# morrislab/rnascan

Hardware: AMD Instinct MI355X
Metric: scored windows/sec (seq+struct, w=12) (higher is better)
Workload: dtype f64

## Files before the change

### include/pfmscan.h

```cpp
#ifndef PFMSCAN_H
#define PFMSCAN_H

#include <stdint.h>

#ifdef __cplusplus
extern "C" {
#endif

#define PFMSCAN_ABI_VERSION 14
#define PFMSCAN_NCODE   8
#define PFMSCAN_SEP     7
#define PFMSCAN_NSTRUCT 7
#define PFMSCAN_MAX_M   64
#define PFMSCAN_MAX_WIDTH 4096

#define PFMSCAN_OK          0
#define PFMSCAN_E_BADARG   -1
#define PFMSCAN_E_BADSHAPE -2
#define PFMSCAN_E_OOM      -3
#define PFMSCAN_E_HIP      -4
#define PFMSCAN_E_CAPACITY -5

#define PFMSCAN_PROFILE_NONE 0
#define PFMSCAN_PROFILE_F32  1
#define PFMSCAN_PROFILE_F64  2

typedef struct pfmscan_ctx pfmscan_ctx;
typedef struct pfmscan_motif pfmscan_motif;

int pfmscan_abi_version(void);

int pfmscan_ctx_create(int device, pfmscan_ctx **out);
// ... 166 lines not shown
int pfmscan_library_sum_thresholds(const double *letter_tables, const double *struct_pssms,
                                   int n_motifs, int m, const double *thr_seq,
                                   const double *thr_sum, double row_sum_max, double *thr_eff_out);

int pfmscan_library_create_letters(pfmscan_ctx *ctx, const double *seq_tables,
                                   const double *struct_tables, int n_motifs, int m,
                                   pfmscan_library **out);
int pfmscan_library_hits_letters_dev(pfmscan_ctx *ctx, pfmscan_library *lib,
                                     const uint8_t *d_codes, const uint8_t *d_codes2, int64_t n_pos,
                                     const double *thr_seq, const double *thr_struct, int64_t capacity,
                                     int64_t *d_hit_pos, int32_t *d_hit_motif, float *d_hit_seq,
                                     double *d_hit_struct, uint64_t *d_hit_count, void *stream);
int pfmscan_library_hits_letters_host(pfmscan_ctx *ctx, pfmscan_library *lib,
                                      const uint8_t *codes, const uint8_t *codes2, int64_t n_pos,
                                      const double *thr_seq, const double *thr_struct, int64_t capacity,
                                      int64_t *hit_pos, int32_t *hit_motif, float *hit_seq,
                                      double *hit_struct, int64_t *n_hits);

int pfmscan_debug_credit_table(const double *letter_table, int m, double thr_seq, int bits,
                               uint16_t *credits, double *slack);

int pfmscan_debug_library8_credits(const double *letter_table, int m, double thr, uint16_t *credits, double *slack);

int pfmscan_debug_credit8_table(const double *letter_table, int m, double thr, uint16_t *credits, int *mode);

#define PFMSCAN_UPLOAD_RUNTIME 0
#define PFMSCAN_UPLOAD_STAGED  1
int pfmscan_set_upload_mode(pfmscan_ctx *ctx, int mode);
int pfmscan_upload_source_file(pfmscan_ctx *ctx, const void *base, size_t length, const char *path, int64_t file_offset);
int pfmscan_upload_source_file_checked(pfmscan_ctx *ctx, const void *base, size_t length, const char *path,
                                       int64_t file_offset, int64_t st_dev, int64_t st_ino, int64_t st_size);

int pfmscan_dotbracket_annotate_dev(pfmscan_ctx *ctx, const uint8_t *d_in, uint8_t *d_out, int64_t n_pos,
                                    const uint8_t *map, int64_t *d_counts, int64_t *first_bad, void *stream);
int pfmscan_dotbracket_stage(pfmscan_ctx *ctx, const uint8_t *codes, int64_t n_pos, int which, const uint8_t *map,
                             int64_t *counts, int64_t *first_bad);
int pfmscan_dotbracket_annotate_host(pfmscan_ctx *ctx, const uint8_t *in, uint8_t *out, int64_t n_pos,
                                     const uint8_t *map, int64_t *counts, int64_t *first_bad);

#define PFMSCAN_MAX_COVER 1024
#define PFMSCAN_AVG_OK         0
#define PFMSCAN_AVG_DOTBRACKET 1
#define PFMSCAN_AVG_UNCOVERED  2
#define PFMSCAN_AVG_COVER      3
#define PFMSCAN_AVG_BAD_TABLE  4
int pfmscan_average_dev(pfmscan_ctx *ctx, const uint8_t *d_letters, int64_t n_letters, const int64_t *d_frag_off,
// ... 84 lines not shown
```

### rnascan_amd/_lib.py

```python
import ctypes
import importlib.util
import os
import sys

import numpy as np

HERE = os.path.dirname(os.path.abspath(__file__))
LIB_PATH = os.environ.get("PFMSCAN_LIB") or os.path.join(HERE, "libpfmscan.so")

OK = 0
E_BADARG, E_BADSHAPE, E_OOM, E_HIP, E_CAPACITY = -1, -2, -3, -4, -5
PROFILE_NONE, PROFILE_F32, PROFILE_F64 = 0, 1, 2
SEP = 7
NCODE = 8
NSTRUCT = 7
MAX_M = 64
MAX_WIDTH = 4096
ABI_VERSION = 14

SYMBOLS = [
    "pfmscan_abi_version", "pfmscan_ctx_create", "pfmscan_ctx_destroy", "pfmscan_last_error",
    "pfmscan_device_info", "pfmscan_synchronize", "pfmscan_motif_create", "pfmscan_motif_destroy",
    "pfmscan_pwm_calculate", "pfmscan_scan_dev", "pfmscan_scan_letters_f64_dev", "pfmscan_hits_dev",
    "pfmscan_scan_host", "pfmscan_scan_letters_f64_host", "pfmscan_hits_host", "pfmscan_time_scan_dev",
    "pfmscan_stage", "pfmscan_scan_staged", "pfmscan_hits_staged", "pfmscan_hits_adaptive_dev",
    "pfmscan_library_create", "pfmscan_library_destroy", "pfmscan_library_info", "pfmscan_library_hits_dev",
    "pfmscan_library_hits_staged", "pfmscan_library_hits_host", "pfmscan_library_hits_pipeline_host", "pfmscan_debug_credit_table",
    "pfmscan_library_create_letters", "pfmscan_library_hits_letters_dev", "pfmscan_library_hits_letters_host", "pfmscan_debug_library8_credits",
    "pfmscan_debug_credit8_table",
    "pfmscan_hits_pipeline_host", "pfmscan_staged_positions",
    "pfmscan_hits_letters_f64_dev", "pfmscan_hits_letters_f64_staged", "pfmscan_hits_letters_f64_host",
    "pfmscan_hits_pair_dev", "pfmscan_stage_codes2", "pfmscan_hits_pair_staged", "pfmscan_hits_pair_host", "pfmscan_round_decimals",
    "pfmscan_set_upload_mode", "pfmscan_upload_source_file", "pfmscan_upload_source_file_checked", "pfmscan_fasta_lone_cr", "pfmscan_count_bytes", "pfmscan_fasta_index", "pfmscan_fasta_ids", "pfmscan_gather_spans", "pfmscan_fasta_encode", "pfmscan_tsv_format", "pfmscan_profile_parse", "pfmscan_tsv_number",
    "pfmscan_place_alloc", "pfmscan_place_free", "pfmscan_place_note", "pfmscan_place_trim",
    "pfmscan_dotbracket_annotate_dev", "pfmscan_dotbracket_stage", "pfmscan_dotbracket_annotate_host",
    "pfmscan_average_dev", "pfmscan_average_host", "pfmscan_average_stage", "pfmscan_fragment_ids",
    "pfmscan_profile_colsums_dev", "pfmscan_profile_colsums_host", "pfmscan_profile_colsums_staged",
    "pfmscan_hits_sum_dev", "pfmscan_hits_sum_staged", "pfmscan_hits_sum_host", "pfmscan_hits_sum_pipeline_host",
    "pfmscan_library_hits_sum_dev", "pfmscan_library_hits_sum_staged", "pfmscan_library_hits_sum_host",
    "pfmscan_profile_row_bound_dev", "pfmscan_profile_row_bound_staged", "pfmscan_library_sum_thresholds",
]
MAX_COVER = 1024
AVG_OK, AVG_DOTBRACKET, AVG_UNCOVERED, AVG_COVER, AVG_BAD_TABLE = range(5)
TSV_CONST, TSV_I64, TSV_F32, TSV_F64, TSV_INDEXED, TSV_FIXED, TSV_WINDOW, TSV_SPAN = range(8)


class TsvColumn(ctypes.Structure):
    _fields_ = [("kind", ctypes.c_int32), ("reserved", ctypes.c_int32), ("data", ctypes.c_void_p),
                ("aux", ctypes.c_void_p), ("blob", ctypes.c_void_p), ("width", ctypes.c_int64)]



# ... 1110 lines not shown
    tj = np.ascontiguousarray(np.broadcast_to(np.asarray(thr_sum, dtype=np.float64), (n,)))
    out = np.empty(n, dtype=np.float64)
    rc = L.pfmscan_library_sum_thresholds(_ptr(T), _ptr(P), n, m, _ptr(ts), _ptr(tj), float(row_sum_max), _ptr(out))
    if rc != OK:
        raise ValueError("pfmscan_library_sum_thresholds: bad argument")
    return out


def library8_credits(letter_table, thr):
    L = load()
    T = np.ascontiguousarray(letter_table, dtype=np.float64)
    if T.ndim != 2 or T.shape[1] != NCODE:
        raise ValueError("letter_table must be [m][8]")
    rows = (T.shape[0] + 3) // 4 * 4
    out = np.zeros((rows, 8), dtype=np.uint16)
    slack = ctypes.c_double(0.0)
    L.pfmscan_debug_library8_credits.argtypes = [ctypes.c_void_p, ctypes.c_int, ctypes.c_double, ctypes.c_void_p, ctypes.POINTER(ctypes.c_double)]
    rc = L.pfmscan_debug_library8_credits(_ptr(T), T.shape[0], float(thr), _ptr(out), ctypes.byref(slack))
    if rc != OK:
        raise ValueError("pfmscan_debug_library8_credits: bad argument")
    return out, slack.value


def credit8_table(letter_table, thr):
    L = load()
    T = np.ascontiguousarray(letter_table, dtype=np.float64)
    if T.ndim != 2 or T.shape[1] != NCODE:
        raise ValueError("letter_table must be [m][8]")
    out = np.zeros((T.shape[0], 8), dtype=np.uint16)
    mode = ctypes.c_int(0)
    rc = L.pfmscan_debug_credit8_table(_ptr(T), T.shape[0], float(thr), _ptr(out), ctypes.byref(mode))
    if rc != OK:
        raise ValueError("pfmscan_debug_credit8_table: bad argument")
    return out, mode.value


def _stream_args(motif, codes, profile):
    if motif.has_letters:
        if codes is None:
            raise ValueError("motif has a letter table: codes required")
        codes = np.ascontiguousarray(codes, dtype=np.uint8)
        n = codes.size
    dt = PROFILE_NONE
    if motif.has_struct:
        if profile is None:
            raise ValueError("motif has a structure PSSM: profile required")
# ... 16 lines not shown
```

### rnascan_amd/build.py

```python
import os
import re
import shutil
import subprocess
import sys
import tempfile
from concurrent.futures import ThreadPoolExecutor

HERE = os.path.dirname(os.path.abspath(__file__))
CSRC = os.path.join(HERE, "csrc")
OBJ = os.path.join(CSRC, "_obj")
LIB = os.path.join(HERE, "libpfmscan.so")
SOURCES = ["pfmscan_kernels.hip", "pfmscan_letters8.hip", "pfmscan_letters_fixed.hip", "pfmscan_api.hip", "pfmscan_hits.hip", "pfmscan_sort.hip", "pfmscan_library.hip", "pfmscan_library_api.hip", "pfmscan_proflib.hip", "pfmscan_profile_fixed.hip", "pfmscan_place.hip",
           "pfmscan_pipeline.hip", "pfmscan_ingest.hip", "pfmscan_upload.hip", "pfmscan_dotbracket.hip", "pfmscan_average.hip", "pfmscan_background.hip", "pfmscan_rowbound.hip"]
HEADERS = ["pfmscan_internal.hpp", "pfmscan_ctx.hpp", "pfmscan_hits.hpp", "pfmscan_hitqueue.hpp", "pfmscan_device.hpp", "pfmscan_profile.hpp", "pfmscan_exact.hpp", os.path.join("..", "..", "include", "pfmscan.h")]
DEPS = SOURCES + HEADERS
FLAGS = ["-O3", "--offload-arch=gfx950", "-std=c++17", "-fPIC", "-fno-fast-math", "-Wall"]


def hipcc_path():
    for cand in (os.environ.get("HIPCC"), shutil.which("hipcc"), "/opt/rocm/bin/hipcc"):
        if cand and os.path.exists(cand):
            return cand
    raise RuntimeError("hipcc not found (set HIPCC or install ROCm under /opt/rocm)")


def stale():
    if not os.path.exists(LIB):
        return True
    t = os.path.getmtime(LIB)
    return any(os.path.getmtime(os.path.join(CSRC, d)) > t for d in DEPS)


def _obj_stale(src, obj):
    if not os.path.exists(obj):
        return True
    t = os.path.getmtime(obj)
    return any(os.path.getmtime(os.path.join(CSRC, d)) > t for d in [src] + HEADERS)
# ... 70 lines not shown
```

### rnascan_amd/csrc/pfmscan_internal.hpp

```cpp
#pragma once
#include <hip/hip_runtime.h>
#include <stdint.h>
#include <atomic>
#include "../../include/pfmscan.h"

namespace pfmscan {

struct CredCache {
    double thr = __builtin_nan("");
    int mode = 0;
    uint16_t cr[16 * 16];
};

struct Cred8Cache {
    double thr = __builtin_nan("");
    int mode = 0;
    uint16_t cr[32 * 8];
};

struct ScanArgs {
    const uint8_t *codes;
    const void *profile;
    int profile_dtype;
    int64_t n_pos;
// ... 142 lines not shown
constexpr int PROFILE_LETTERS2 = 100;
__host__ __device__ constexpr int lib8_rows(int m) { return (m + 3) / 4 * 4; }
size_t lib8_group_bytes(int m);
size_t lib8_lds_bytes(int m, int ng);
int lib8_pick_ng(int want_groups, int max_groups);
hipError_t launch_library8(const LibArgs &a, int n_cu, hipStream_t stream);

struct ProfLibArgs {
    const void *profile;
    int profile_dtype;
    int64_t n_pos;
    const double *pssm;
    const double *thr;
    double struct_band;
    const int32_t *finite;
    int n_motifs, m, motif_base;
    int64_t pos_offset;
    int64_t capacity;
    int hit_shards;
    int64_t *hit_pos;
    int32_t *hit_motif;
    double *hit_struct;
    unsigned long long *hit_count;
};
hipError_t launch_profile_library(const ProfLibArgs &a, hipStream_t stream);
int64_t profile_library_tile();

hipError_t sort_temp_bytes(int64_t total, int key_bits, size_t *bytes);
hipError_t launch_gather_sorted(const GatherArgs &g, hipStream_t stream);

}
```

### rnascan_amd/csrc/pfmscan_library_api.hip

```cpp
#include <algorithm>
#include <cmath>
#include <cstdlib>
#include <cstring>
#include <new>
#include <string>
#include <vector>

#include "pfmscan_hits.hpp"

using namespace pfmscan;

namespace {

struct LibPass {
    int motif_base = 0, n_real = 0, nmp = 0, ng = 0;
    int ng_real = 0;
    size_t pairs_off = 0;
    size_t letters_off = 0;
    size_t pssm_off = 0;
    size_t thr_off = 0;
};

}

double pfmscan::build_credits(const double *pairsum, int npair, double thr, uint16_t *out, int bits, int nent)
{
    std::fill(out, out + (size_t)npair * nent, (uint16_t)0);
    if (thr == INFINITY) return 0.0;
    const int half = 1 << (bits - 1);
    const int V = std::min(half - 1, (half - 1) / std::max(npair - 1, 1));
    const int X = (npair - 1) * V + 1;
// ... 39 lines not shown
        }
    return q * npair;
}

void pfmscan::pair_sums(const double *T, int m, double *out)
{
    const int npair = (m + 1) / 2;
    for (int t = 0; t < npair; ++t)
        for (int c0 = 0; c0 < 4; ++c0)
            for (int c1 = 0; c1 < 4; ++c1)
                out[t * 16 + (c0 | c1 << 2)] = T[(2 * t) * 8 + c0] + (2 * t + 1 < m ? T[(2 * t + 1) * 8 + c1] : 0.0);
}

struct pfmscan_library {
    pfmscan_ctx *ctx = nullptr;
    int n = 0, m = 0, npair = 0, np_bucket = 8;
    bool has_struct = false;
    bool has_letters = true;
    bool pair = false;
    bool letters8 = false;
    std::vector<double> rows8;
    double *d_pssm_rows = nullptr;
    int32_t *d_finite = nullptr;
    bool all_finite = false;
    double struct_band = 0.0;
    std::vector<double> pairsum;
    std::vector<LibPass> passes;
    uint16_t *d_pairs = nullptr;
    double *d_letters = nullptr, *d_pssm = nullptr, *d_thr = nullptr;
    size_t pairs_elems = 0, thr_elems = 0;
    std::vector<uint16_t> h_pairs;
    std::vector<double> h_thr;
    std::vector<double> cur_seq, cur_struct, eps;
    std::vector<double> h_letters, h_pssm;
    std::vector<double> band;
    std::vector<double> cur_eff, cur_sum;
    bool thr_valid = false;
};

static int lib_fail(pfmscan_ctx *ctx, int code, const std::string &msg) { return fail(ctx, code, msg); }

extern "C" {

static int create_seq_library(pfmscan_ctx *ctx, const double *letter_tables, const double *struct_pssms, int ncol, int n_motifs, int m,
                              pfmscan_library **out);

// ... 7 lines not shown
        return lib_fail(ctx, PFMSCAN_E_BADSHAPE, "PFM width " + std::to_string(m) + " outside 1.." + std::to_string(PFMSCAN_MAX_M));
    if (!letter_tables) {
        HIP_TRY(ctx, hipSetDevice(ctx->device));
        pfmscan_library *lib = new (std::nothrow) pfmscan_library();
        if (!lib) return lib_fail(ctx, PFMSCAN_E_OOM, "out of host memory");
        lib->ctx = ctx;
        lib->n = n_motifs;
        lib->m = m;
        lib->has_struct = true;
        lib->has_letters = false;
        for (int k = 0; k < n_motifs; ++k) lib->struct_band = std::max(lib->struct_band, struct_band(struct_pssms + (size_t)k * m * 7, m));
        std::vector<int32_t> fin((size_t)n_motifs, 1);
        for (int k = 0; k < n_motifs; ++k)
            for (int i = 0; i < m * 7; ++i)
                if (!std::isfinite(struct_pssms[(size_t)k * m * 7 + i])) fin[(size_t)k] = 0;
        if (std::getenv("PFMSCAN_FORCE_GENERIC")) std::fill(fin.begin(), fin.end(), 0);
        const size_t cells = (size_t)n_motifs * m * 7;
        hipError_t e = hipMalloc((void **)&lib->d_pssm_rows, cells * 8);
        if (e == hipSuccess) e = hipMemcpy(lib->d_pssm_rows, struct_pssms, cells * 8, hipMemcpyHostToDevice);
        if (e == hipSuccess) e = hipMalloc((void **)&lib->d_finite, (size_t)n_motifs * 4);
        if (e == hipSuccess) e = hipMemcpy(lib->d_finite, fin.data(), (size_t)n_motifs * 4, hipMemcpyHostToDevice);
        if (e == hipSuccess) e = hipMalloc((void **)&lib->d_thr, (size_t)n_motifs * 8);
        lib->thr_elems = (size_t)n_motifs;
        if (e != hipSuccess) {
            pfmscan_library_destroy(lib);
            return fail_hip(ctx, e, "uploading the library tables");
        }
        *out = lib;
        return PFMSCAN_OK;
    }
    return create_seq_library(ctx, letter_tables, struct_pssms, 7, n_motifs, m, out);
}

}

static int create_seq_library(pfmscan_ctx *ctx, const double *letter_tables, const double *struct_pssms, int ncol, int n_motifs, int m,
                              pfmscan_library **out)
{
    for (int64_t i = 0; i < (int64_t)n_motifs * m; ++i)
        for (int c = 4; c < 8; ++c)
            if (!std::isnan(letter_tables[i * 8 + c]))
                return lib_fail(ctx, PFMSCAN_E_BADSHAPE, "library scans need a 4-letter alphabet: columns 4..7 of every letter table must be NaN");
    HIP_TRY(ctx, hipSetDevice(ctx->device));
    pfmscan_library *lib = new (std::nothrow) pfmscan_library();
    if (!lib) return lib_fail(ctx, PFMSCAN_E_OOM, "out of host memory");
    lib->ctx = ctx;
// ... 151 lines not shown
{
    if (!ctx || !out || !struct_tables) return lib_fail(ctx, PFMSCAN_E_BADARG, "pfmscan_library_create_letters: NULL argument");
    *out = nullptr;
    if (n_motifs < 1 || n_motifs > 65535) return lib_fail(ctx, PFMSCAN_E_BADSHAPE, "library size outside 1..65535");
    if (m < 1 || m > PFMSCAN_MAX_M)
        return lib_fail(ctx, PFMSCAN_E_BADSHAPE, "PFM width " + std::to_string(m) + " outside 1.." + std::to_string(PFMSCAN_MAX_M));
    for (int64_t i = 0; i < (int64_t)n_motifs * m; ++i)
        if (!std::isnan(struct_tables[i * 8 + 7]))
            return lib_fail(ctx, PFMSCAN_E_BADSHAPE, "column 7 of every letter table must be NaN (the foreign code)");
    if (seq_tables) return create_seq_library(ctx, seq_tables, struct_tables, 8, n_motifs, m, out);
    return create_letters8_library(ctx, struct_tables, n_motifs, m, out);
}

void pfmscan_library_destroy(pfmscan_library *lib)
{
    if (!lib) return;
    if (lib->ctx) (void)hipSetDevice(lib->ctx->device);
    if (lib->d_pairs) (void)hipFree(lib->d_pairs);
    if (lib->d_letters) (void)hipFree(lib->d_letters);
    if (lib->d_pssm) (void)hipFree(lib->d_pssm);
    if (lib->d_thr) (void)hipFree(lib->d_thr);
    if (lib->d_pssm_rows) (void)hipFree(lib->d_pssm_rows);
    if (lib->d_finite) (void)hipFree(lib->d_finite);
    delete lib;
}

int pfmscan_debug_credit_table(const double *letter_table, int m, double thr_seq, int bits, uint16_t *credits, double *slack)
{
    if (!letter_table || !credits || m < 1 || m > PFMSCAN_MAX_M || std::isnan(thr_seq)) return PFMSCAN_E_BADARG;
    if (bits == 0) bits = lib_credit_bits(lib_np_bucket(m));
    if (bits != 10 && bits != 16) return PFMSCAN_E_BADARG;
    const int npair = (m + 1) / 2;
    std::vector<double> ps((size_t)npair * 16);
    pair_sums(letter_table, m, ps.data());
    const double s = build_credits(ps.data(), npair, thr_seq, credits, bits);
    if (slack) *slack = s;
    return PFMSCAN_OK;
}

int pfmscan_debug_library8_credits(const double *letter_table, int m, double thr, uint16_t *credits, double *slack)
{
    if (!letter_table || !credits || m < 1 || m > 32 || std::isnan(thr)) return PFMSCAN_E_BADARG;
    const int rows = lib8_rows(m);
    std::vector<double> r8((size_t)rows * 8, 0.0);
    for (int j = 0; j < m; ++j)
        for (int c = 0; c < 8; ++c) r8[(size_t)j * 8 + c] = std::isnan(letter_table[j * 8 + c]) ? -INFINITY : letter_table[j * 8 + c];
    const double s = build_credits(r8.data(), rows, thr, credits, 16, 8);
    if (slack) *slack = s;
    return PFMSCAN_OK;
}

int pfmscan_library_info(const pfmscan_library *lib, int *n_motifs, int *m, int *n_passes, int *motifs_per_pass, double *max_eps)
{
    if (!lib) return PFMSCAN_E_BADARG;
    if (n_motifs) *n_motifs = lib->n;
    if (m) *m = lib->m;
    const bool tabled = lib->has_letters || lib->letters8;
    if (n_passes) *n_passes = tabled ? (int)lib->passes.size() : 1;
    if (motifs_per_pass) *motifs_per_pass = !tabled ? lib->n : (lib->passes.empty() ? 0 : lib->passes[0].nmp);
    if (max_eps) {
        double mx = 0.0;
        for (double v : lib->eps) mx = std::max(mx, v);
        *max_eps = lib->thr_valid ? mx : NAN;
    }
    return PFMSCAN_OK;
}

}

static int lib_set_thresholds(pfmscan_ctx *ctx, pfmscan_library *lib, const double *thr_seq, const double *thr_struct, hipStream_t st,
                              const double *thr_sum = nullptr, double row_sum_max = INFINITY)
{
    const int n = lib->n, npair = lib->npair;
    if (!lib->has_letters && !lib->letters8) {
        for (int k = 0; k < n; ++k)
            if (std::isnan(thr_struct[k])) return lib_fail(ctx, PFMSCAN_E_BADARG, "NaN threshold");
        if (lib->thr_valid && std::equal(thr_struct, thr_struct + n, lib->cur_struct.begin())) return PFMSCAN_OK;
        HIP_TRY(ctx, hipStreamSynchronize(st));
        lib->h_thr.assign(thr_struct, thr_struct + n);
        HIP_TRY(ctx, hipMemcpyAsync(lib->d_thr, lib->h_thr.data(), (size_t)n * 8, hipMemcpyHostToDevice, st));
        lib->cur_struct.assign(thr_struct, thr_struct + n);
        lib->eps.assign((size_t)n, 0.0);
        lib->thr_valid = true;
        return PFMSCAN_OK;
    }
    if (lib->letters8) {
        const int rows = lib->npair;
        for (int k = 0; k < n; ++k) {
            if (std::isnan(thr_struct[k])) return lib_fail(ctx, PFMSCAN_E_BADARG, "NaN threshold");
            if (thr_struct[k] == -INFINITY)
                return lib_fail(ctx, PFMSCAN_E_BADARG, "library hits need a finite threshold (every window would be a hit; use the all-scores entry points)");
        }
        if (lib->thr_valid && std::equal(thr_struct, thr_struct + n, lib->cur_struct.begin())) return PFMSCAN_OK;
        HIP_TRY(ctx, hipStreamSynchronize(st));
        lib->thr_valid = false;
        lib->h_pairs.assign(lib->pairs_elems, (uint16_t)0);
        lib->h_thr.assign(lib->thr_elems, 0.0);
        lib->eps.assign((size_t)n, 0.0);
        std::vector<uint16_t> cr((size_t)rows * 8);
        uint32_t *words = reinterpret_cast<uint32_t *>(lib->h_pairs.data());
        for (const LibPass &ps : lib->passes)
            for (int l = 0; l < ps.nmp; ++l) {
                const int g = l / 8, slot = l % 8;
// ... 120 lines not shown
            }
        return PFMSCAN_OK;
    }
    if (!lib->has_letters) {
        ProfLibArgs a;
        std::memset(&a, 0, sizeof(a));
        a.profile = d_profile;
        a.profile_dtype = profile_dtype;
        a.n_pos = n_pos;
        a.pssm = lib->d_pssm_rows;
        a.thr = lib->d_thr;
        a.struct_band = lib->struct_band;
        a.finite = lib->d_finite;
        a.n_motifs = lib->n;
        a.m = lib->m;
        a.motif_base = 0;
        a.pos_offset = pos_offset;
        a.capacity = sink.shard_cap;
        a.hit_shards = sink.shards;
        a.hit_pos = sink.pos;
        a.hit_motif = sink.motif;
        a.hit_struct = sink.st;
        a.hit_count = sink.count;
        hipError_t e = launch_profile_library(a, st);
        if (e != hipSuccess) return fail_hip(ctx, e, "launch k_profile_lib");
        return PFMSCAN_OK;
    }
    const LibPass &first_pass = lib->passes[0];
    bool teams = lib->has_struct && !lib->pair && lib->passes.size() > 1 && n_pos >= (int64_t)8 * ctx->n_cu * LIB_SEG &&
                 ctx->n_cu >= 16 && !std::getenv("PFMSCAN_LIB_SEQUENTIAL");
    for (const LibPass &ps : lib->passes) teams = teams && ps.ng == first_pass.ng;
    const int64_t max_span = (int64_t)1 << 31;
    for (int64_t base = 0; base < n_pos; base += max_span) {
        const int64_t span_segs = (std::min<int64_t>(max_span, n_pos - base) + LIB_SEG - 1) / LIB_SEG;
        const size_t per_launch = teams && span_segs >= ctx->n_cu ? 4 : 1;
        for (size_t p0 = 0; p0 < lib->passes.size(); p0 += per_launch) {
            const LibPass &ps = lib->passes[p0];
            const size_t nt = std::min(per_launch, lib->passes.size() - p0);
            LibArgs a;
            std::memset(&a, 0, sizeof(a));
            a.ng_real = ps.ng_real;
            {
                static const int sort_env = std::getenv("PFMSCAN_LIB_SORT") ? std::atoi(std::getenv("PFMSCAN_LIB_SORT")) : 0;
                a.sort_batches = sort_env;
            }
            if (nt > 1) {
// ... 366 lines not shown
```

### rnascan_amd/csrc/pfmscan_proflib.hip

```cpp
#include <float.h>
#include <math.h>

#include "pfmscan_internal.hpp"
#include "pfmscan_exact.hpp"
#include "pfmscan_hitqueue.hpp"

namespace pfmscan {

constexpr int PL_LANES = 256;
constexpr int PL_GROUPS = 4;
constexpr int PL_BLOCK = PL_LANES * PL_GROUPS;
#ifndef PL_V_OVERRIDE
#define PL_V_OVERRIDE 5
#endif
constexpr int PL_V = PL_V_OVERRIDE;
constexpr int PL_NS = PL_V + 1;
constexpr int PL_UNROLL = (PL_NS % 2) ? 2 * PL_NS : PL_NS;
constexpr int PL_TILE = PL_LANES * PL_V;
#ifndef PL_WAIT_FIRST
#define PL_WAIT_FIRST 1
#endif
#ifndef PL_STAGGER
#define PL_STAGGER 0
#endif
#ifndef PL_INTERLEAVE
#define PL_INTERLEAVE 0
#endif
constexpr int PL_QCAP = 128;

typedef uint32_t pl_u32x4 __attribute__((ext_vector_type(4)));
typedef double pl_f64x2 __attribute__((ext_vector_type(2)));

__device__ __forceinline__ double pl_nan_to_num(double d)
{
    double c = fmin(fmax(d, -DBL_MAX), DBL_MAX);
    return (d != d) ? 0.0 : c;
}

__host__ __device__ constexpr int pl_tile_vals(int m) { return ((PL_TILE + m) * 7 + 3) / 4 * 4; }
__host__ __device__ constexpr int pl_tile_bytes(int m) { return pl_tile_vals(m) * 8; }
__host__ __device__ constexpr int pl_queue_bytes() { return (PL_BLOCK / 64) * PL_QCAP * (8 + 4); }

__device__ __forceinline__ double pl_window_slow(const double *tile, int local, const double *__restrict__ pssm, int m)
{
    double score = 0.0;
#pragma unroll 1
    for (int j = 0; j < m; ++j) {
        const double *r = tile + (local + j) * 7;
        double d = r[0] * pssm[j * 7];
#pragma unroll 1
        for (int k = 1; k < 7; ++k) d = fma(r[k], pssm[j * 7 + k], d);
        score += pl_nan_to_num(d);
    }
    return score;
}

template <bool FINITE>
__device__ __forceinline__ void pl_score_motif(const double *tile, const double *__restrict__ pssm, const double *__restrict__ pssm_next,
                                               int m, int la, double (&acc)[PL_V], double (&P)[7])
{
    constexpr int V = PL_V, NS = PL_NS;
    const volatile __attribute__((address_space(3))) double *vt = (const volatile __attribute__((address_space(3))) double *)tile;
    double rows[NS][7];
#pragma unroll
    for (int s = 0; s < V; ++s) {
#pragma unroll
        for (int k = 0; k < 7; ++k) rows[s][k] = vt[(la + s) * 7 + k];
        acc[s] = 0.0;
    }
#if defined(PL_ABLATE) && (PL_ABLATE & 2)
#pragma unroll
    for (int k = 0; k < 7; ++k) rows[V][k] = rows[0][k];
#endif
    double Q[7];
    auto step = [&](const int uu, const int j) __attribute__((always_inline)) {
        const int u = uu % NS;
        double (&C)[7] = (uu & 1) ? Q : P;
        double (&N)[7] = (uu & 1) ? P : Q;
#if PL_WAIT_FIRST
        __builtin_amdgcn_s_waitcnt(0xC07F);
        __builtin_amdgcn_sched_barrier(0);
#endif
        const double *nrow = (j + 1 < m) ? pssm + (j + 1) * 7 : pssm_next;
        const __attribute__((address_space(4))) double *prow = (const __attribute__((address_space(4))) double *)nrow;
#if defined(PL_ABLATE) && (PL_ABLATE & 1)
        (void)prow;
#pragma unroll
        for (int k = 0; k < 7; ++k) N[k] = C[k];
#else
#pragma unroll
        for (int k = 0; k < 7; ++k) N[k] = prow[k];
#endif
#if defined(PL_ABLATE) && (PL_ABLATE & 2)
#else
#pragma unroll
        for (int k = 0; k < 7; ++k) rows[(u + V) % NS][k] = vt[(la + j + V) * 7 + k];
#endif
        if (FINITE) {
#pragma unroll
            for (int k = 0; k < 7; ++k) {
#pragma unroll
                for (int v = 0; v < V; ++v) acc[v] = fma(rows[(u + v) % NS][k], C[k], acc[v]);
            }
        } else {
#pragma unroll
            for (int v = 0; v < V; ++v) {
                const int slot = (u + v) % NS;
                double d = rows[slot][0] * C[0];
#pragma unroll
                for (int k = 1; k < 7; ++k) d = fma(rows[slot][k], C[k], d);
                acc[v] += pl_nan_to_num(d);
            }
        }
    };
    int j0 = 0;
#pragma unroll 1
    for (; j0 + PL_UNROLL <= m; j0 += PL_UNROLL) {
#pragma unroll
        for (int uu = 0; uu < PL_UNROLL; ++uu) step(uu, j0 + uu);
// ... 130 lines not shown
                if (__builtin_amdgcn_ballot_w64(pass) == 0) continue;
                if (pass && acc[v] <= t_hi) {
                    acc[v] = struct_window_rounded(tile + (la + v) * 7, m, [&](int j, int c) { return pssm[j * 7 + c]; });
                    pass = acc[v] > t;
                }
                const unsigned long long mk = __builtin_amdgcn_ballot_w64(pass);
                if (mk) {
                    if (qn + 64 > PL_QCAP) flush();
                    if (pass) {
                        const int slot = qn + (int)__builtin_amdgcn_mbcnt_hi((uint32_t)(mk >> 32), __builtin_amdgcn_mbcnt_lo((uint32_t)mk, 0u));
                        q_sc[slot] = acc[v];
                        q_wm[slot] = ((uint32_t)(la + v) << 16) | (uint32_t)k;
                    }
                    qn += __popcll(mk);
                }
            }
        }
        k = kn;
        if (kn < nm) kn = (int)__builtin_amdgcn_readfirstlane(draw());
    }
    if (qn > 0) flush();
}

int64_t profile_library_tile() { return PL_TILE; }

hipError_t launch_profile_library(const ProfLibArgs &a, hipStream_t stream)
{
    if (a.n_pos <= 0 || a.n_motifs <= 0) return hipSuccess;
    if (a.n_motifs > 65536 || a.m < 1 || a.m > PFMSCAN_MAX_M) return hipErrorInvalidValue;
    const unsigned grid = (unsigned)((a.n_pos + PL_TILE - 1) / PL_TILE);
    const size_t lds = (size_t)pl_tile_bytes(a.m) + pl_queue_bytes() + 16;
    static std::atomic<uint64_t> done_f{0}, done_d{0};
    if (a.profile_dtype == PFMSCAN_PROFILE_F64) {
        hipError_t e = allow_dynamic_lds(reinterpret_cast<const void *>(k_profile_lib<double>), done_d, 160 * 1024);
        if (e != hipSuccess) return e;
        hipLaunchKernelGGL(k_profile_lib<double>, dim3(grid), dim3(PL_BLOCK), lds, stream, a);
    } else {
        hipError_t e = allow_dynamic_lds(reinterpret_cast<const void *>(k_profile_lib<float>), done_f, 160 * 1024);
        if (e != hipSuccess) return e;
        hipLaunchKernelGGL(k_profile_lib<float>, dim3(grid), dim3(PL_BLOCK), lds, stream, a);
    }
    return hipGetLastError();
}

}
```

Baseline: 150.4 billion.

## Add int8 dot-product prescreen to profile library kernel before exact f64 scoring

Adds a screening variant of the structure-profile library kernel. Each motif's PSSM is quantised to int8 and each profile row to 8-bit, and an sdot4 integer score with a conservative threshold (padded by slack and band) rejects (window, motif) pairs. Surviving pairs are batched and rescored exactly in f64. It is on by default for motifs whose estimated survival rate is low, so most f64 FMAs are replaced by cheap integer dot products. The cost is extra LDS for the quantised rows, plus the risk that the conservative bounds are wrong or that divergent survivor batches add overhead.

```diff
diff --git a/include/pfmscan.h b/include/pfmscan.h
--- a/include/pfmscan.h
+++ b/include/pfmscan.h
@@ -7,7 +7,7 @@
 extern "C" {
 #endif
 
-#define PFMSCAN_ABI_VERSION 14
+#define PFMSCAN_ABI_VERSION 15
 #define PFMSCAN_NCODE   8
 #define PFMSCAN_SEP     7
 #define PFMSCAN_NSTRUCT 7
@@ -220,6 +220,9 @@
 
 int pfmscan_debug_library8_credits(const double *letter_table, int m, double thr, uint16_t *credits, double *slack);
 
+int pfmscan_debug_proflib_screen(const double *struct_pssms, int n_motifs, int m, const double *thr, int8_t *pq, double *scale,
+                                 int32_t *tq, double *slack, int32_t *screened, const float *probe, int64_t n_probe, uint8_t *probe_q);
+
 int pfmscan_debug_credit8_table(const double *letter_table, int m, double thr, uint16_t *credits, int *mode);
 
 #define PFMSCAN_UPLOAD_RUNTIME 0
diff --git a/rnascan_amd/_lib.py b/rnascan_amd/_lib.py
--- a/rnascan_amd/_lib.py
+++ b/rnascan_amd/_lib.py
@@ -16,7 +16,7 @@
 NSTRUCT = 7
 MAX_M = 64
 MAX_WIDTH = 4096
-ABI_VERSION = 14
+ABI_VERSION = 15
 
 SYMBOLS = [
     "pfmscan_abi_version", "pfmscan_ctx_create", "pfmscan_ctx_destroy", "pfmscan_last_error",
@@ -27,7 +27,7 @@
     "pfmscan_library_create", "pfmscan_library_destroy", "pfmscan_library_info", "pfmscan_library_hits_dev",
     "pfmscan_library_hits_staged", "pfmscan_library_hits_host", "pfmscan_library_hits_pipeline_host", "pfmscan_debug_credit_table",
     "pfmscan_library_create_letters", "pfmscan_library_hits_letters_dev", "pfmscan_library_hits_letters_host", "pfmscan_debug_library8_credits",
-    "pfmscan_debug_credit8_table",
+    "pfmscan_debug_credit8_table", "pfmscan_debug_proflib_screen",
     "pfmscan_hits_pipeline_host", "pfmscan_staged_positions",
     "pfmscan_hits_letters_f64_dev", "pfmscan_hits_letters_f64_staged", "pfmscan_hits_letters_f64_host",
     "pfmscan_hits_pair_dev", "pfmscan_stage_codes2", "pfmscan_hits_pair_staged", "pfmscan_hits_pair_host", "pfmscan_round_decimals",
@@ -1184,6 +1184,29 @@
     return out, slack.value
 
 
+def proflib_screen(struct_pssms, thr, probe=None):
+    L = load()
+    P = np.ascontiguousarray(struct_pssms, dtype=np.float64)
+    if P.ndim != 3 or P.shape[2] != NSTRUCT:
+        raise ValueError("struct_pssms must be [n][m][7]")
+    n, m = P.shape[:2]
+    t = np.ascontiguousarray(np.broadcast_to(np.asarray(thr, dtype=np.float64), (n,)))
+    out = {"pq": np.zeros((n, m, 8), dtype=np.int8), "scale": np.zeros(n), "tq": np.zeros(n, dtype=np.int32),
+           "slack": np.zeros(n), "screened": np.zeros(n, dtype=np.int32), "probe_q": None}
+    pr = None
+    if probe is not None:
+        pr = np.ascontiguousarray(probe, dtype=np.float32).reshape(-1)
+        out["probe_q"] = np.zeros(pr.size, dtype=np.uint8)
+    L.pfmscan_debug_proflib_screen.argtypes = [ctypes.c_void_p, ctypes.c_int, ctypes.c_int, ctypes.c_void_p, ctypes.c_void_p, ctypes.c_void_p,
+                                               ctypes.c_void_p, ctypes.c_void_p, ctypes.c_void_p, ctypes.c_void_p, ctypes.c_int64, ctypes.c_void_p]
+    rc = L.pfmscan_debug_proflib_screen(_ptr(P), n, m, _ptr(t), _ptr(out["pq"]), _ptr(out["scale"]), _ptr(out["tq"]), _ptr(out["slack"]),
+                                        _ptr(out["screened"]), None if pr is None else _ptr(pr), 0 if pr is None else pr.size,
+                                        None if pr is None else _ptr(out["probe_q"]))
+    if rc != OK:
+        raise ValueError("pfmscan_debug_proflib_screen: bad argument")
+    return out
+
+
 def credit8_table(letter_table, thr):
     L = load()
     T = np.ascontiguousarray(letter_table, dtype=np.float64)
diff --git a/rnascan_amd/build.py b/rnascan_amd/build.py
--- a/rnascan_amd/build.py
+++ b/rnascan_amd/build.py
@@ -12,7 +12,7 @@
 LIB = os.path.join(HERE, "libpfmscan.so")
 SOURCES = ["pfmscan_kernels.hip", "pfmscan_letters8.hip", "pfmscan_letters_fixed.hip", "pfmscan_api.hip", "pfmscan_hits.hip", "pfmscan_sort.hip", "pfmscan_library.hip", "pfmscan_library_api.hip", "pfmscan_proflib.hip", "pfmscan_profile_fixed.hip", "pfmscan_place.hip",
            "pfmscan_pipeline.hip", "pfmscan_ingest.hip", "pfmscan_upload.hip", "pfmscan_dotbracket.hip", "pfmscan_average.hip", "pfmscan_background.hip", "pfmscan_rowbound.hip"]
-HEADERS = ["pfmscan_internal.hpp", "pfmscan_ctx.hpp", "pfmscan_hits.hpp", "pfmscan_hitqueue.hpp", "pfmscan_device.hpp", "pfmscan_profile.hpp", "pfmscan_exact.hpp", os.path.join("..", "..", "include", "pfmscan.h")]
+HEADERS = ["pfmscan_internal.hpp", "pfmscan_ctx.hpp", "pfmscan_hits.hpp", "pfmscan_hitqueue.hpp", "pfmscan_device.hpp", "pfmscan_profile.hpp", "pfmscan_exact.hpp", "pfmscan_proflib_screen.hpp", os.path.join("..", "..", "include", "pfmscan.h")]
 DEPS = SOURCES + HEADERS
 FLAGS = ["-O3", "--offload-arch=gfx950", "-std=c++17", "-fPIC", "-fno-fast-math", "-Wall"]
 
diff --git a/rnascan_amd/csrc/pfmscan_internal.hpp b/rnascan_amd/csrc/pfmscan_internal.hpp
--- a/rnascan_amd/csrc/pfmscan_internal.hpp
+++ b/rnascan_amd/csrc/pfmscan_internal.hpp
@@ -188,6 +188,11 @@
     int32_t *hit_motif;
     double *hit_struct;
     unsigned long long *hit_count;
+    const int8_t *pq;
+    const int32_t *tq;
+    const int32_t *screened;
+    int screen_level;
+    unsigned long long *screen_stats;
 };
 hipError_t launch_profile_library(const ProfLibArgs &a, hipStream_t stream);
 int64_t profile_library_tile();
diff --git a/rnascan_amd/csrc/pfmscan_library_api.hip b/rnascan_amd/csrc/pfmscan_library_api.hip
--- a/rnascan_amd/csrc/pfmscan_library_api.hip
+++ b/rnascan_amd/csrc/pfmscan_library_api.hip
@@ -1,5 +1,6 @@
 #include <algorithm>
 #include <cmath>
+#include <cstdio>
 #include <cstdlib>
 #include <cstring>
 #include <new>
@@ -7,6 +8,7 @@
 #include <vector>
 
 #include "pfmscan_hits.hpp"
+#include "pfmscan_proflib_screen.hpp"
 
 using namespace pfmscan;
 
@@ -92,6 +94,14 @@
     std::vector<double> rows8;
     double *d_pssm_rows = nullptr;
     int32_t *d_finite = nullptr;
+    std::vector<ScreenMotif> screen;
+    std::vector<int8_t> h_pq;
+    std::vector<int32_t> h_tq;
+    int8_t *d_pq = nullptr;
+    int32_t *d_tq = nullptr;
+    int screened_max = 0;
+    bool any_screened = false;
+    unsigned long long *d_screen_stats = nullptr;
     bool all_finite = false;
     double struct_band = 0.0;
     std::vector<double> pairsum;
@@ -145,6 +155,17 @@
         if (e == hipSuccess) e = hipMemcpy(lib->d_finite, fin.data(), (size_t)n_motifs * 4, hipMemcpyHostToDevice);
         if (e == hipSuccess) e = hipMalloc((void **)&lib->d_thr, (size_t)n_motifs * 8);
         lib->thr_elems = (size_t)n_motifs;
+        lib->screen.resize((size_t)n_motifs);
+        lib->h_pq.resize((size_t)n_motifs * m * 8);
+        for (int k = 0; k < n_motifs; ++k)
+            lib->screen[(size_t)k] = screen_motif(struct_pssms + (size_t)k * m * 7, m, lib->h_pq.data() + (size_t)k * m * 8);
+        if (e == hipSuccess) e = hipMalloc((void **)&lib->d_pq, lib->h_pq.size());
+        if (e == hipSuccess) e = hipMemcpy(lib->d_pq, lib->h_pq.data(), lib->h_pq.size(), hipMemcpyHostToDevice);
+        if (e == hipSuccess) e = hipMalloc((void **)&lib->d_tq, (size_t)n_motifs * 2 * 4);
+        if (e == hipSuccess && std::getenv("PFMSCAN_PROFLIB_STATS")) {
+            e = hipMalloc((void **)&lib->d_screen_stats, 16);
+            if (e == hipSuccess) e = hipMemset(lib->d_screen_stats, 0, 16);
+        }
         if (e != hipSuccess) {
             pfmscan_library_destroy(lib);
             return fail_hip(ctx, e, "uploading the library tables");
@@ -342,6 +363,14 @@
     if (lib->d_thr) (void)hipFree(lib->d_thr);
     if (lib->d_pssm_rows) (void)hipFree(lib->d_pssm_rows);
     if (lib->d_finite) (void)hipFree(lib->d_finite);
+    if (lib->d_pq) (void)hipFree(lib->d_pq);
+    if (lib->d_tq) (void)hipFree(lib->d_tq);
+    if (lib->d_screen_stats) {
+        unsigned long long st[2] = {0, 0};
+        if (hipMemcpy(st, lib->d_screen_stats, 16, hipMemcpyDeviceToHost) == hipSuccess)
+            std::fprintf(stderr, "pfmscan: k_profile_lib_screen: %llu survivors of %llu screened (window, motif) pairs\n", st[0], st[1]);
+        (void)hipFree(lib->d_screen_stats);
+    }
     delete lib;
 }
 
@@ -367,6 +396,25 @@
         for (int c = 0; c < 8; ++c) r8[(size_t)j * 8 + c] = std::isnan(letter_table[j * 8 + c]) ? -INFINITY : letter_table[j * 8 + c];
     const double s = build_credits(r8.data(), rows, thr, credits, 16, 8);
     if (slack) *slack = s;
+    return PFMSCAN_OK;
+}
+
+int pfmscan_debug_proflib_screen(const double *struct_pssms, int n_motifs, int m, const double *thr, int8_t *pq, double *scale,
+                                 int32_t *tq, double *slack, int32_t *screened, const float *probe, int64_t n_probe, uint8_t *probe_q)
+{
+    if (!struct_pssms || !thr || !pq || !scale || !tq || !slack || !screened || n_motifs < 1 || m < 1 || m > PFMSCAN_MAX_M) return PFMSCAN_E_BADARG;
+    if (n_probe < 0 || (n_probe > 0 && (!probe || !probe_q))) return PFMSCAN_E_BADARG;
+    double band = 0.0;
+    for (int k = 0; k < n_motifs; ++k) band = std::max(band, struct_band(struct_pssms + (size_t)k * m * 7, m));
+    for (int k = 0; k < n_motifs; ++k) {
+        const ScreenMotif sm = screen_motif(struct_pssms + (size_t)k * m * 7, m, pq + (size_t)k * m * 8);
+        scale[k] = sm.scale;
+        slack[k] = sm.slack;
+        tq[k] = sm.ok ? screen_threshold(sm, thr[k], band) : INT32_MIN;
+        screened[k] = !sm.ok ? 0 : (screen_survival(pq + (size_t)k * m * 8, m, tq[k]) <= SCREEN_DENSE ? 1 : 2);
+    }
+    for (int64_t i = 0; i < n_probe; ++i)
+        probe_q[i] = (probe[i] >= 0.0f && probe[i] <= 1.0f) ? (uint8_t)screen_quantise(probe[i]) : (uint8_t)255;
     return PFMSCAN_OK;
 }
 
@@ -399,6 +447,20 @@
         HIP_TRY(ctx, hipStreamSynchronize(st));
         lib->h_thr.assign(thr_struct, thr_struct + n);
         HIP_TRY(ctx, hipMemcpyAsync(lib->d_thr, lib->h_thr.data(), (size_t)n * 8, hipMemcpyHostToDevice, st));
+        lib->h_tq.assign((size_t)n * 2, 0);
+        lib->any_screened = false;
+        lib->screened_max = 0;
+        for (int k = 0; k < n; ++k) {
+            const ScreenMotif &sm = lib->screen[(size_t)k];
+            if (!sm.ok) continue;
+            const int32_t tq = screen_threshold(sm, thr_struct[k], lib->struct_band);
+            lib->h_tq[(size_t)k] = tq;
+            const bool on = screen_survival(lib->h_pq.data() + (size_t)k * lib->m * 8, lib->m, tq) <= SCREEN_DENSE;
+            lib->h_tq[(size_t)(n + k)] = on ? 1 : 2;
+            lib->any_screened = lib->any_screened || on;
+            lib->screened_max = std::max(lib->screened_max, on ? 1 : 2);
+        }
+        HIP_TRY(ctx, hipMemcpyAsync(lib->d_tq, lib->h_tq.data(), (size_t)n * 2 * 4, hipMemcpyHostToDevice, st));
         lib->cur_struct.assign(thr_struct, thr_struct + n);
         lib->eps.assign((size_t)n, 0.0);
         lib->thr_valid = true;
@@ -565,6 +627,15 @@
         a.hit_motif = sink.motif;
         a.hit_struct = sink.st;
         a.hit_count = sink.count;
+        const char *screen_env = std::getenv("PFMSCAN_PROFLIB_SCREEN");
+        const int screen_level = screen_env ? std::atoi(screen_env) : 1;
+        if (screen_level >= 2 ? lib->screened_max > 0 : (screen_level == 1 && lib->any_screened)) {
+            a.screen_level = screen_level >= 2 ? 2 : 1;
+            a.pq = lib->d_pq;
+            a.tq = lib->d_tq;
+            a.screened = lib->d_tq + lib->n;
+            a.screen_stats = lib->d_screen_stats;
+        }
         hipError_t e = launch_profile_library(a, st);
         if (e != hipSuccess) return fail_hip(ctx, e, "launch k_profile_lib");
         return PFMSCAN_OK;
diff --git a/rnascan_amd/csrc/pfmscan_proflib.hip b/rnascan_amd/csrc/pfmscan_proflib.hip
--- a/rnascan_amd/csrc/pfmscan_proflib.hip
+++ b/rnascan_amd/csrc/pfmscan_proflib.hip
@@ -4,6 +4,7 @@
 #include "pfmscan_internal.hpp"
 #include "pfmscan_exact.hpp"
 #include "pfmscan_hitqueue.hpp"
+#include "pfmscan_proflib_screen.hpp"
 
 namespace pfmscan {
 
@@ -41,31 +42,32 @@
 __host__ __device__ constexpr int pl_tile_bytes(int m) { return pl_tile_vals(m) * 8; }
 __host__ __device__ constexpr int pl_queue_bytes() { return (PL_BLOCK / 64) * PL_QCAP * (8 + 4); }
 
-__device__ __forceinline__ double pl_window_slow(const double *tile, int local, const double *__restrict__ pssm, int m)
+template <typename TT>
+__device__ __forceinline__ double pl_window_slow(const TT *tile, int local, const double *__restrict__ pssm, int m)
 {
     double score = 0.0;
 #pragma unroll 1
     for (int j = 0; j < m; ++j) {
-        const double *r = tile + (local + j) * 7;
-        double d = r[0] * pssm[j * 7];
-#pragma unroll 1
-        for (int k = 1; k < 7; ++k) d = fma(r[k], pssm[j * 7 + k], d);
+        const TT *r = tile + (local + j) * 7;
+        double d = (double)r[0] * pssm[j * 7];
+#pragma unroll 1
+        for (int k = 1; k < 7; ++k) d = fma((double)r[k], pssm[j * 7 + k], d);
         score += pl_nan_to_num(d);
     }
     return score;
 }
 
-template <bool FINITE>
-__device__ __forceinline__ void pl_score_motif(const double *tile, const double *__restrict__ pssm, const double *__restrict__ pssm_next,
+template <bool FINITE, typename TT>
+__device__ __forceinline__ void pl_score_motif(const TT *tile, const double *__restrict__ pssm, const double *__restrict__ pssm_next,
                                                int m, int la, double (&acc)[PL_V], double (&P)[7])
 {
     constexpr int V = PL_V, NS = PL_NS;
-    const volatile __attribute__((address_space(3))) double *vt = (const volatile __attribute__((address_space(3))) double *)tile;
+    const volatile __attribute__((address_space(3))) TT *vt = (const volatile __attribute__((address_space(3))) TT *)tile;
     double rows[NS][7];
 #pragma unroll
     for (int s = 0; s < V; ++s) {
 #pragma unroll
-        for (int k = 0; k < 7; ++k) rows[s][k] = vt[(la + s) * 7 + k];
+        for (int k = 0; k < 7; ++k) rows[s][k] = (double)vt[(la + s) * 7 + k];
         acc[s] = 0.0;
     }
 #if defined(PL_ABLATE) && (PL_ABLATE & 2)
@@ -94,7 +96,7 @@
 #if defined(PL_ABLATE) && (PL_ABLATE & 2)
 #else
 #pragma unroll
-        for (int k = 0; k < 7; ++k) rows[(u + V) % NS][k] = vt[(la + j + V) * 7 + k];
+        for (int k = 0; k < 7; ++k) rows[(u + V) % NS][k] = (double)vt[(la + j + V) * 7 + k];
 #endif
         if (FINITE) {
 #pragma unroll
@@ -271,6 +273,281 @@
     if (qn > 0) flush();
 }
 
+constexpr int PS_SVCAP = 128;
+
+typedef int32_t ps_i32x2 __attribute__((ext_vector_type(2)));
+
+template <typename PROF_T> __host__ __device__ constexpr int ps_raw_bytes(int m) { return pl_tile_vals(m) * (int)sizeof(PROF_T); }
+__host__ __device__ constexpr int ps_q_bytes(int m) { return (PL_TILE + m) * 8; }
+__host__ __device__ constexpr int ps_sv_bytes() { return (PL_BLOCK / 64) * PS_SVCAP * 4; }
+
+__device__ __forceinline__ void ps_screen_motif(const ps_i32x2 *qrows, const int8_t *__restrict__ pq, int m, int la, int32_t (&acc)[PL_V])
+{
+    constexpr int V = PL_V, NS = PL_NS;
+    const __attribute__((address_space(3))) ps_i32x2 *qt = (const __attribute__((address_space(3))) ps_i32x2 *)qrows;
+    const __attribute__((address_space(4))) ps_i32x2 *pr = (const __attribute__((address_space(4))) ps_i32x2 *)pq;
+    ps_i32x2 rows[NS];
+#pragma unroll
+    for (int s = 0; s < V; ++s) {
+        rows[s] = qt[la + s];
+        acc[s] = 0;
+    }
+    auto step = [&](const int uu, const int j) __attribute__((always_inline)) {
+        const int u = uu % NS;
+        const ps_i32x2 c = pr[j];
+        rows[(u + V) % NS] = qt[la + j + V];
+#pragma unroll
+        for (int v = 0; v < V; ++v) {
+            const int slot = (u + v) % NS;
+            acc[v] = __builtin_amdgcn_sdot4(rows[slot].x, c.x, acc[v], false);
+            acc[v] = __builtin_amdgcn_sdot4(rows[slot].y, c.y, acc[v], false);
+        }
+    };
+    int j0 = 0;
+#pragma unroll 1
+    for (; j0 + NS <= m; j0 += NS) {
+#pragma unroll
+        for (int uu = 0; uu < NS; ++uu) step(uu, j0 + uu);
+    }
+#pragma unroll
+    for (int uu = 0; uu < NS - 1; ++uu) {
+        if (j0 + uu < m) step(uu, j0 + uu);
+    }
+}
+
+template <typename PROF_T>
+__global__ __launch_bounds__(PL_BLOCK) void k_profile_lib_screen(const ProfLibArgs a)
+{
+    constexpr int V = PL_V;
+    constexpr int PER = 16 / (int)sizeof(PROF_T);
+    typedef PROF_T vec_t __attribute__((ext_vector_type(PER)));
+    extern __shared__ __align__(16) unsigned char smem[];
+    const int m = a.m;
+    PROF_T *tile = reinterpret_cast<PROF_T *>(smem);
+    ps_i32x2 *qrows = reinterpret_cast<ps_i32x2 *>(smem + ps_raw_bytes<PROF_T>(m));
+    unsigned char *rest = smem + ps_raw_bytes<PROF_T>(m) + ps_q_bytes(m);
+    const int lane = threadIdx.x & 63;
+    const int wave = __builtin_amdgcn_readfirstlane(threadIdx.x >> 6);
+    const int group = wave / (PL_LANES / 64);
+    double *q_sc = reinterpret_cast<double *>(rest) + wave * PL_QCAP;
+    uint32_t *q_wm = reinterpret_cast<uint32_t *>(rest + (PL_BLOCK / 64) * PL_QCAP * 8) + wave * PL_QCAP;
+    uint32_t *sv = reinterpret_cast<uint32_t *>(rest + pl_queue_bytes()) + wave * PS_SVCAP;
+    uint32_t *tickets = reinterpret_cast<uint32_t *>(rest + pl_queue_bytes() + ps_sv_bytes());
+    const int64_t n_pos = a.n_pos;
+    const int64_t tile0 = (int64_t)blockIdx.x * PL_TILE;
+
+    {
+        const int nval = pl_tile_vals(m);
+        const int64_t e0 = tile0 * 7, e_end = n_pos * 7;
+        const PROF_T *__restrict__ src = reinterpret_cast<const PROF_T *>(a.profile) + e0;
+        for (int i = threadIdx.x * PER; i < nval; i += PL_BLOCK * PER) {
+            vec_t v;
+            if (e0 + i + PER <= e_end) {
+                v = __builtin_nontemporal_load(reinterpret_cast<const vec_t *>(src + i));
+            } else {
+#pragma unroll
+                for (int e = 0; e < PER; ++e) v[e] = (e0 + i + e < e_end) ? src[i + e] : (PROF_T)0;
+            }
+            *reinterpret_cast<vec_t *>(tile + i) = v;
+        }
+    }
+    if (threadIdx.x < PL_LANES / 64) tickets[threadIdx.x] = PL_GROUPS;
+    uint32_t *tile_flag = tickets + PL_LANES / 64;
+    if (threadIdx.x == 0) *tile_flag = 0u;
+    __syncthreads();
+    int bad = 0;
+    for (int r = threadIdx.x; r < PL_TILE + m; r += PL_BLOCK) {
+        uint32_t w[2] = {0u, 0u};
+#pragma unroll
+        for (int c = 0; c < 7; ++c) {
+            const PROF_T f = tile[r * 7 + c];
+            const bool in = f >= (PROF_T)0 && f <= (PROF_T)1;
+            bad |= !in;
+            w[c >> 2] |= (in ? screen_quantise(f) & 0x7Fu : 0u) << (8 * (c & 3));
+        }
+        qrows[r] = ps_i32x2{(int32_t)w[0], (int32_t)w[1]};
+    }
+    if (bad) *tile_flag = 1u;
+    __syncthreads();
+    const bool flagged = __builtin_amdgcn_readfirstlane(*tile_flag) != 0u;
+
+    const HitShard shard{a.hit_count, a.hit_shards, a.capacity};
+    const unsigned long long shard_off = shard.off();
+    int qn = 0;
+    auto flush = [&]() {
+        __builtin_amdgcn_fence(__ATOMIC_RELEASE, "wavefront");
+        __builtin_amdgcn_wave_barrier();
+        __builtin_amdgcn_fence(__ATOMIC_ACQUIRE, "wavefront");
+        const unsigned long long base = shard.reserve_wave(qn);
+        for (int i = lane; i < qn; i += 64) {
+            const unsigned long long slot = base + (unsigned long long)i;
+            if (shard.in_range(slot)) {
+                const uint32_t wm = q_wm[i];
+                a.hit_pos[shard_off + slot] = tile0 + (int64_t)(wm >> 16) + a.pos_offset;
+                a.hit_motif[shard_off + slot] = a.motif_base + (int32_t)(wm & 0xFFFFu);
+                a.hit_struct[shard_off + slot] = q_sc[i];
+            }
+        }
+        __builtin_amdgcn_fence(__ATOMIC_RELEASE, "wavefront");
+        __builtin_amdgcn_wave_barrier();
+        qn = 0;
+    };
+    auto push_hits = [&](bool pass, int local, int mo, double score) {
+        const unsigned long long mk = __builtin_amdgcn_ballot_w64(pass);
+        if (mk) {
+            if (qn + 64 > PL_QCAP) flush();
+            if (pass) {
+                const int slot = qn + (int)__builtin_amdgcn_mbcnt_hi((uint32_t)(mk >> 32), __builtin_amdgcn_mbcnt_lo((uint32_t)mk, 0u));
+                q_sc[slot] = score;
+                q_wm[slot] = ((uint32_t)local << 16) | (uint32_t)mo;
+            }
+            qn += __popcll(mk);
+        }
+    };
+
+    const int la = (threadIdx.x & (PL_LANES - 1)) * V;
+    const int64_t live_all = n_pos - m + 1 - tile0;
+    const int live_n = live_all < 0 ? 0 : (live_all > PL_TILE ? PL_TILE : (int)live_all);
+    const __attribute__((address_space(4))) double *thr = (const __attribute__((address_space(4))) double *)a.thr;
+    const __attribute__((address_space(4))) int32_t *finite = (const __attribute__((address_space(4))) int32_t *)a.finite;
+    const __attribute__((address_space(4))) int32_t *tq = (const __attribute__((address_space(4))) int32_t *)a.tq;
+    const __attribute__((address_space(4))) int32_t *screened = (const __attribute__((address_space(4))) int32_t *)a.screened;
+
+    int sn = 0;
+    auto exact_batch = [&](int at, int cnt) {
+        __builtin_amdgcn_fence(__ATOMIC_RELEASE, "wavefront");
+        __builtin_amdgcn_wave_barrier();
+        __builtin_amdgcn_fence(__ATOMIC_ACQUIRE, "wavefront");
+        const bool act = lane < cnt;
+        const uint32_t e = act ? sv[at + lane] : 0u;
+        const int local = (int)(e >> 16), mo = (int)(e & 0xFFFFu);
+        double acc = 0.0;
+        bool pass = false;
+        if (act) {
+            const double *__restrict__ ps = a.pssm + (size_t)mo * m * 7;
+            const double t = a.thr[mo];
+            if (a.finite[mo]) {
+#pragma unroll 1
+                for (int j = 0; j < m; ++j) {
+#pragma unroll
+                    for (int c = 0; c < 7; ++c) acc = fma((double)tile[(local + j) * 7 + c], ps[j * 7 + c], acc);
+                }
+                if (!(fabs(acc) <= DBL_MAX)) acc = pl_window_slow(tile, local, ps, m);
+            } else {
+#pragma unroll 1
+                for (int j = 0; j < m; ++j) {
+                    double d = (double)tile[(local + j) * 7] * ps[j * 7];
+#pragma unroll
+                    for (int c = 1; c < 7; ++c) d = fma((double)tile[(local + j) * 7 + c], ps[j * 7 + c], d);
+                    acc += pl_nan_to_num(d);
+                }
+            }
+            pass = acc > t - a.struct_band;
+            if (pass && acc <= t + a.struct_band) {
+                acc = struct_window_rounded(tile + local * 7, m, [&](int j, int c) { return ps[j * 7 + c]; });
+                pass = acc > t;
+            }
+        }
+        push_hits(pass, local, mo, acc);
+        __builtin_amdgcn_fence(__ATOMIC_RELEASE, "wavefront");
+        __builtin_amdgcn_wave_barrier();
+    };
+
+    uint32_t *ticket = tickets + (wave & (PL_LANES / 64 - 1));
+    auto draw = [&]() -> uint32_t {
+        uint32_t v = 0;
+        if (lane == 0) v = atomicAdd(ticket, 1u);
+        return v;
+    };
+    const int nm = a.n_motifs;
+    int k = group;
+    int kn = nm;
+    double P[7] = {0.0, 0.0, 0.0, 0.0, 0.0, 0.0, 0.0};
+    bool p_valid = false;
+    uint32_t n_surv = 0, n_pairs = 0;
+    const int wave_first = (wave & (PL_LANES / 64 - 1)) * 64 * V;
+    const int wave_live = live_n - wave_first < 0 ? 0 : (live_n - wave_first > 64 * V ? 64 * V : live_n - wave_first);
+    if (k < nm) kn = (int)__builtin_amdgcn_readfirstlane(draw());
+#pragma unroll 1
+    while (k < nm) {
+        const int scr_k = screened[k];
+        const bool scr = !flagged && scr_k != 0 && scr_k <= a.screen_level;
+        if (scr) {
+            int32_t I[V];
+            ps_screen_motif(qrows, a.pq + (size_t)k * m * 8, m, la, I);
+            const int32_t t = tq[k];
+            bool keep[V], any = false;
+#pragma unroll
+            for (int v = 0; v < V; ++v) {
+                keep[v] = (la + v < live_n) && (I[v] >= t);
+                any = any || keep[v];
+            }
+            n_pairs += (uint32_t)wave_live;
+            if (__builtin_amdgcn_ballot_w64(any) != 0) {
+#pragma unroll
+                for (int v = 0; v < V; ++v) {
+                    const unsigned long long mk = __builtin_amdgcn_ballot_w64(keep[v]);
+                    if (mk == 0) continue;
+                    if (keep[v])
+                        sv[sn + (int)__builtin_amdgcn_mbcnt_hi((uint32_t)(mk >> 32), __builtin_amdgcn_mbcnt_lo((uint32_t)mk, 0u))] =
+                            ((uint32_t)(la + v) << 16) | (uint32_t)k;
+                    sn += __popcll(mk);
+                    n_surv += (uint32_t)__popcll(mk);
+                    if (sn >= 64) {
+                        exact_batch(sn - 64, 64);
+                        sn -= 64;
+                    }
+                }
+            }
+            p_valid = false;
+        } else {
+            const double *pssm = a.pssm + (size_t)k * m * 7;
+            const int kc = kn < nm ? kn : k;
+            const double *pssm_next = a.pssm + (size_t)kc * m * 7;
+            if (!p_valid) {
+                const __attribute__((address_space(4))) double *p0 = (const __attribute__((address_space(4))) double *)pssm;
+#pragma unroll
+                for (int c = 0; c < 7; ++c) P[c] = p0[c];
+            }
+            const double t = thr[k];
+            const int fin = finite[k];
+            double acc[V];
+            if (fin)
+                pl_score_motif<true>(tile, pssm, pssm_next, m, la, acc, P);
+            else
+                pl_score_motif<false>(tile, pssm, pssm_next, m, la, acc, P);
+            p_valid = kn < nm;
+            const double t_lo = t - a.struct_band, t_hi = t + a.struct_band;
+            bool maybe[V], any = false;
+#pragma unroll
+            for (int v = 0; v < V; ++v) {
+                maybe[v] = (la + v < live_n) && (acc[v] > t_lo);
+                any = any || maybe[v];
+            }
+            if (__builtin_expect(__builtin_amdgcn_ballot_w64(any) != 0, 0)) {
+#pragma unroll
+                for (int v = 0; v < V; ++v) {
+                    bool pass = maybe[v];
+                    if (__builtin_amdgcn_ballot_w64(pass) == 0) continue;
+                    if (pass && acc[v] <= t_hi) {
+                        acc[v] = struct_window_rounded(tile + (la + v) * 7, m, [&](int j, int c) { return pssm[j * 7 + c]; });
+                        pass = acc[v] > t;
+                    }
+                    push_hits(pass, la + v, k, acc[v]);
+                }
+            }
+        }
+        k = kn;
+        if (kn < nm) kn = (int)__builtin_amdgcn_readfirstlane(draw());
+    }
+    if (sn > 0) exact_batch(0, sn);
+    if (qn > 0) flush();
+    if (a.screen_stats && lane == 0) {
+        atomicAdd(a.screen_stats, (unsigned long long)n_surv);
+        atomicAdd(a.screen_stats + 1, (unsigned long long)n_pairs);
+    }
+}
+
 int64_t profile_library_tile() { return PL_TILE; }
 
 hipError_t launch_profile_library(const ProfLibArgs &a, hipStream_t stream)
@@ -279,7 +556,20 @@
     if (a.n_motifs > 65536 || a.m < 1 || a.m > PFMSCAN_MAX_M) return hipErrorInvalidValue;
     const unsigned grid = (unsigned)((a.n_pos + PL_TILE - 1) / PL_TILE);
     const size_t lds = (size_t)pl_tile_bytes(a.m) + pl_queue_bytes() + 16;
-    static std::atomic<uint64_t> done_f{0}, done_d{0};
+    static std::atomic<uint64_t> done_f{0}, done_d{0}, done_sf{0}, done_sd{0};
+    if (a.pq) {
+        const size_t rest = (size_t)ps_q_bytes(a.m) + pl_queue_bytes() + ps_sv_bytes() + 32;
+        if (a.profile_dtype == PFMSCAN_PROFILE_F64) {
+            hipError_t e = allow_dynamic_lds(reinterpret_cast<const void *>(k_profile_lib_screen<double>), done_sd, 160 * 1024);
+            if (e != hipSuccess) return e;
+            hipLaunchKernelGGL(k_profile_lib_screen<double>, dim3(grid), dim3(PL_BLOCK), ps_raw_bytes<double>(a.m) + rest, stream, a);
+        } else {
+            hipError_t e = allow_dynamic_lds(reinterpret_cast<const void *>(k_profile_lib_screen<float>), done_sf, 160 * 1024);
+            if (e != hipSuccess) return e;
+            hipLaunchKernelGGL(k_profile_lib_screen<float>, dim3(grid), dim3(PL_BLOCK), ps_raw_bytes<float>(a.m) + rest, stream, a);
+        }
+        return hipGetLastError();
+    }
     if (a.profile_dtype == PFMSCAN_PROFILE_F64) {
         hipError_t e = allow_dynamic_lds(reinterpret_cast<const void *>(k_profile_lib<double>), done_d, 160 * 1024);
         if (e != hipSuccess) return e;
diff --git a/rnascan_amd/csrc/pfmscan_proflib_screen.hpp b/rnascan_amd/csrc/pfmscan_proflib_screen.hpp
--- /dev/null
+++ b/rnascan_amd/csrc/pfmscan_proflib_screen.hpp
@@ -0,0 +1,98 @@
+#pragma once
+#include <math.h>
+#include <stdint.h>
+#include <cmath>
+#include <vector>
+#include <hip/hip_runtime.h>
+
+#include "pfmscan_exact.hpp"
+
+namespace pfmscan {
+
+constexpr double SCREEN_CELL_MAX = 1e100;
+constexpr double SCREEN_DENSE = 1.0 / 32.0;
+
+template <typename T> __host__ __device__ __forceinline__ uint32_t screen_quantise(T f)
+{
+#pragma clang fp contract(off)
+    const T p = f * (T)127;
+    T q = floor(p);
+    const T e = fma(f, (T)127, -p);
+    if (q == p && e < (T)0) q -= (T)1;
+    return (uint32_t)(int32_t)q;
+}
+
+struct ScreenMotif {
+    bool ok = false;
+    double scale = 1.0;
+    double slack = 0.0;
+};
+
+inline ScreenMotif screen_motif(const double *pssm, int m, int8_t *pq)
+{
+    ScreenMotif s;
+    for (int i = 0; i < m * 8; ++i) pq[i] = 0;
+    double mx = 0.0;
+    for (int i = 0; i < m * 7; ++i) {
+        const double p = pssm[i];
+        if (std::isnan(p) || p == INFINITY) return s;
+        if (p == -INFINITY) continue;
+        if (std::fabs(p) > SCREEN_CELL_MAX) return s;
+        mx = std::max(mx, std::fabs(p));
+    }
+    s.scale = mx > 0.0 ? next_up(mx / 126.0) : 1.0;
+    if (!(s.scale > 0.0) || !std::isfinite(s.scale)) s.scale = 1.0;
+    double pos = 0.0;
+    for (int j = 0; j < m; ++j) {
+        bool dead = false;
+        for (int c = 0; c < 7; ++c) dead = dead || pssm[j * 7 + c] == -INFINITY;
+        if (dead) continue;
+        for (int c = 0; c < 7; ++c) {
+            const double p = pssm[j * 7 + c];
+            double q = std::ceil(p / s.scale);
+            while (next_down(q * s.scale) < p) q += 1.0;
+            if (q > 127.0 || q < -127.0) return ScreenMotif();
+            pq[j * 8 + c] = (int8_t)q;
+            if (p > 0.0) pos = next_up(pos + p);
+        }
+    }
+    s.slack = next_up(pos / 127.0);
+    s.ok = true;
+    return s;
+}
+
+inline int32_t screen_threshold(const ScreenMotif &s, double t, double band)
+{
+    if (std::isnan(t) || t == -INFINITY) return INT32_MIN;
+    if (t == INFINITY) return INT32_MAX;
+    double x = next_down(t - 2.0 * band);
+    x = next_down(x - s.slack);
+    double y = next_down(x * 127.0);
+    y = next_down(y / s.scale);
+    if (std::isnan(y)) return INT32_MIN;
+    y = std::floor(y);
+    if (y <= (double)INT32_MIN) return INT32_MIN;
+    if (y >= (double)INT32_MAX) return INT32_MAX;
+    return (int32_t)y;
+}
+
+inline double screen_survival(const int8_t *pq, int m, int32_t tq)
+{
+    if (tq == INT32_MIN) return 1.0;
+    if (tq == INT32_MAX) return 0.0;
+    double mean = 0.0, var = 0.0;
+    for (int j = 0; j < m; ++j) {
+        double s1 = 0.0, s2 = 0.0;
+        for (int c = 0; c < 7; ++c) {
+            s1 += (double)pq[j * 8 + c];
+            s2 += (double)pq[j * 8 + c] * (double)pq[j * 8 + c];
+        }
+        mean += 2.0 * s1 / 7.0;
+        var += 2.0 * (s2 / 7.0 - (s1 / 7.0) * (s1 / 7.0));
+    }
+    const double x = 2.0 * (double)tq / 127.0 - mean;
+    if (!(var > 0.0)) return x <= 0.0 ? 1.0 : 0.0;
+    return 0.5 * std::erfc(x / std::sqrt(2.0 * var));
+}
+
+}
```

New measurement: 150.7 billion, median of 6. Within noise of the previous version (+0.1%).
